# lazear/sage

Measured on NVIDIA H100. Metric: spectra/sec, higher is better.
Workload: dtype f32

## Files before the change

include/sage_b200.h:

```cpp
#ifndef SAGE_B200_H
#define SAGE_B200_H

#include <stddef.h>
#include <stdint.h>

#ifdef __cplusplus
extern "C" {
#endif

#define SAGE_B200_OK 0
#define SAGE_B200_EINVAL (-1)
#define SAGE_B200_ECUDA (-2)
#define SAGE_B200_ENOTMS2 (-3)
#define SAGE_B200_ENOPRECURSOR (-4)
#define SAGE_B200_ELIMIT (-5)

typedef struct sage_b200_db sage_b200_db;
typedef struct sage_b200_scorer sage_b200_scorer;

enum { SAGE_B200_TOL_PPM = 0, SAGE_B200_TOL_PCT = 1, SAGE_B200_TOL_DA = 2 };
typedef struct { int32_t kind; float lo, hi; } sage_b200_tolerance;

enum { SAGE_B200_KIND_A = 0, SAGE_B200_KIND_B = 1, SAGE_B200_KIND_C = 2, SAGE_B200_KIND_X = 3, SAGE_B200_KIND_Y = 4, SAGE_B200_KIND_Z = 5 };

// ... 101 lines not shown
int sage_b200_db_export_index(const sage_b200_db* db, uint32_t* fragment_peptide, float* fragment_mz, float* bucket_min);
void sage_b200_db_destroy(sage_b200_db* db);

int sage_b200_scorer_create(const sage_b200_db* db, const sage_b200_scorer_params* params, sage_b200_scorer** out);
void sage_b200_scorer_destroy(sage_b200_scorer* scorer);
int sage_b200_scorer_set_option(sage_b200_scorer* scorer, const char* name, int64_t value);

int sage_b200_score_batch(sage_b200_scorer* scorer, const sage_b200_spectra* spectra, sage_b200_feature* features, uint32_t* counts,
                          sage_b200_fragment* fragments, uint64_t fragment_capacity, uint64_t* fragments_used);

int sage_b200_score_batch_multi(sage_b200_scorer* const* scorers, int n_scorers, const sage_b200_spectra* spectra, sage_b200_feature* features,
                                uint32_t* counts);

int sage_b200_bind_thread_to_device(int device);

int sage_b200_quick_score(sage_b200_scorer* scorer, const sage_b200_spectra* spectra, int prefilter_low_memory, uint8_t* keep);

int sage_b200_batch_upload(sage_b200_scorer* scorer, const sage_b200_spectra* spectra);
int sage_b200_batch_run(sage_b200_scorer* scorer);
int sage_b200_batch_download(sage_b200_scorer* scorer, sage_b200_feature* features, uint32_t* counts);

int64_t sage_b200_initial_hits(sage_b200_scorer* scorer, const sage_b200_spectra* one_spectrum, uint16_t* matched, uint32_t* peptide,
                               uint8_t* charge, int8_t* isotope_error, uint64_t cap, uint64_t* matched_peaks, uint64_t* scored_candidates);

int sage_b200_counters_get(const sage_b200_scorer* scorer, sage_b200_counters* out);

typedef struct { uint64_t take_top_n; uint8_t deisotope; float min_deisotope_mz; } sage_b200_processor_params;
typedef struct {
    uint64_t n;
    const uint64_t* peak_offsets;
    const float* mz;
    const float* intensity;
    const uint8_t* precursor_charge;
    const uint8_t* level;
} sage_b200_raw_spectra;
int sage_b200_process_spectra(int device, const sage_b200_processor_params* processor, const sage_b200_raw_spectra* raw, uint64_t* out_peak_offsets,
                              float* out_masses, float* out_intensities, float* out_tic);

int sage_b200_find_reporter_ions(int device, uint64_t n, const uint64_t* peak_offsets, const float* masses, const float* intensities, const float* labels,
                                 uint64_t n_labels, sage_b200_tolerance label_tolerance, float* out);

int sage_b200_host_log_variant(void);
int sage_b200_host_log1pf_exact(void);
int sage_b200_device_log(int device, int variant, const double* x, uint64_t n, double* out);

typedef struct sage_b200_lfq sage_b200_lfq;
// ... 172 lines not shown
```

sage_b200/api.py:

```python
from __future__ import annotations

import ctypes as C
import os
from dataclasses import dataclass, field

import numpy as np

from .build import build_library, library_path

PPM, PCT, DA = 0, 1, 2
KIND = {"a": 0, "b": 1, "c": 2, "x": 3, "y": 4, "z": 5}


class SageB200Error(RuntimeError):
    def __init__(self, code: int, message: str):
        super().__init__(f"sage_b200 error {code}: {message}")
        self.code = code
        self.message = message


class CTol(C.Structure):
    _fields_ = [("kind", C.c_int32), ("lo", C.c_float), ("hi", C.c_float)]


# ... 28 lines not shown
COUNTER_U64 = ["spectra", "peaks", "queries", "tasks", "pages", "entries_scanned", "matched_fragments", "candidates_scored", "peptide_record_floats",
               "psms", "wide_queries", "pep_queries", "pep_fallbacks", "wide_overflows", "algorithmic_bytes", "prelim_bytes", "score_bytes", "h2d_bytes", "d2h_bytes", "kernel_launches", "chunk_retries"]
COUNTER_F32 = ["ms_total", "ms_h2d", "ms_setup", "ms_prelim", "ms_score", "ms_d2h", "ms_prelim_count", "ms_wall"]


class CCounters(C.Structure):
    _fields_ = [(n, C.c_uint64) for n in COUNTER_U64] + [(n, C.c_float) for n in COUNTER_F32]


FEATURE_DTYPE = np.dtype([
    ("spectrum", "<u4"), ("peptide_idx", "<u4"), ("peptide_len", "<u4"), ("rank", "<u4"), ("label", "<i4"), ("expmass", "<f4"), ("calcmass", "<f4"),
    ("charge", "<u4"), ("rt", "<f4"), ("ims", "<f4"), ("delta_mass", "<f4"), ("isotope_error", "<f4"), ("average_ppm", "<f4"), ("_pad0", "<u4"),
    ("hyperscore", "<f8"), ("delta_next", "<f8"), ("delta_best", "<f8"), ("matched_peaks", "<u4"), ("longest_b", "<u4"), ("longest_y", "<u4"),
    ("longest_y_pct", "<f4"), ("missed_cleavages", "<u4"), ("matched_intensity_pct", "<f4"), ("scored_candidates", "<u4"), ("ms2_intensity", "<f4"),
    ("poisson", "<f8"), ("fragment_offset", "<u4"), ("fragment_count", "<u4"),
])
assert FEATURE_DTYPE.itemsize == 128
FRAGMENT_DTYPE = np.dtype([("kind", "<i4"), ("charge", "<i4"), ("ordinal", "<i4"), ("intensity", "<f4"), ("mz_calculated", "<f4"),
                           ("mz_experimental", "<f4")])

EXPORTED_SYMBOLS = [
    "sage_b200_device_count", "sage_b200_db_create", "sage_b200_db_build", "sage_b200_db_get_info", "sage_b200_db_export_index", "sage_b200_db_destroy",
    "sage_b200_scorer_create", "sage_b200_scorer_destroy", "sage_b200_scorer_set_option", "sage_b200_score_batch", "sage_b200_batch_upload", "sage_b200_batch_run",
    "sage_b200_batch_download", "sage_b200_score_batch_multi", "sage_b200_quick_score", "sage_b200_initial_hits", "sage_b200_counters_get",
    "sage_b200_process_spectra", "sage_b200_find_reporter_ions", "sage_b200_host_alloc", "sage_b200_host_free", "sage_b200_last_error",
    "sage_b200_host_log_variant", "sage_b200_host_log1pf_exact", "sage_b200_device_log", "sage_b200_bind_thread_to_device", "sage_b200_host_alloc_blocks",
    "sage_b200_lfq_create", "sage_b200_lfq_add_ms1", "sage_b200_lfq_integrate", "sage_b200_lfq_get_info", "sage_b200_lfq_export", "sage_b200_lfq_destroy",
    "sage_b200_spectrum_fdr", "sage_b200_kde_build", "sage_b200_device_math", "sage_b200_predict_rt",
    "sage_b200_picked_fdr", "sage_b200_picked_precursor", "sage_b200_competition_keys", "sage_b200_protein_groups", "sage_b200_bipartite_cover",
]

_lib = None


def load_library(build: bool = True):
    global _lib
    if _lib is not None:
        return _lib
    path = library_path()
    if not os.path.exists(path):
        if not build:
            raise FileNotFoundError(f"{path} not built; run `python -m sage_b200.build`")
        build_library()
    lib = C.CDLL(path)
    for s in EXPORTED_SYMBOLS:
        getattr(lib, s)
    lib.sage_b200_host_alloc.restype = C.c_void_p
    lib.sage_b200_host_alloc.argtypes = [C.c_size_t]
    lib.sage_b200_host_free.argtypes = [C.c_void_p]
    lib.sage_b200_host_alloc_blocks.restype = C.c_void_p
    lib.sage_b200_host_alloc_blocks.argtypes = [C.c_size_t, C.c_void_p, C.c_int]
    lib.sage_b200_last_error.restype = C.c_size_t
    lib.sage_b200_initial_hits.restype = C.c_int64
    lib.sage_b200_db_destroy.argtypes = [C.c_void_p]
    lib.sage_b200_scorer_destroy.argtypes = [C.c_void_p]
    lib.sage_b200_lfq_destroy.argtypes = [C.c_void_p]
    _lib = lib
    return lib


def _last_error() -> str:
    buf = C.create_string_buffer(2048)
    load_library().sage_b200_last_error(buf, C.c_size_t(2048))
    return buf.value.decode(errors="replace")


def _check(rc: int):
    if rc != 0:
        raise SageB200Error(int(rc), _last_error())


def device_count() -> int:
    return int(load_library().sage_b200_device_count())


def bind_thread_to_device(device: int) -> int:
# ... 339 lines not shown
            keep = np.zeros(self.db.info["n_peptides"], np.uint8)
        keep_c = np.ascontiguousarray(keep, dtype=np.uint8)
        kl: list = []
        cs = batch._c(kl)
        _check(load_library().sage_b200_quick_score(self._h, C.byref(cs), C.c_int(int(prefilter_low_memory)), _ptr(keep_c)))
        return keep_c

    def score(self, spectrum: ProcessedSpectrum):
        out, counts = self.score_batch(SpectraBatch.from_spectra([spectrum]))
        return out[:counts[0]]

    def initial_hits(self, batch: SpectraBatch):
        assert len(batch) == 1
        cap = 256
        m, p = np.zeros(cap, np.uint16), np.zeros(cap, np.uint32)
        c, i = np.zeros(cap, np.uint8), np.zeros(cap, np.int8)
        mp, scd = C.c_uint64(0), C.c_uint64(0)
        keep: list = []
        cs = batch._c(keep)
        n = load_library().sage_b200_initial_hits(self._h, C.byref(cs), _ptr(m), _ptr(p), _ptr(c), _ptr(i), C.c_uint64(cap), C.byref(mp), C.byref(scd))
        if n < 0:
            raise SageB200Error(int(n), _last_error())
        return dict(matched=m[:n].copy(), peptide=p[:n].copy(), charge=c[:n].copy(), iso=i[:n].copy(), matched_peaks=mp.value, scored_candidates=scd.value)

    def counters(self) -> dict:
        cc = CCounters()
        _check(load_library().sage_b200_counters_get(self._h, C.byref(cc)))
        return {k: getattr(cc, k) for k, _ in CCounters._fields_}


def score_batch_multi(scorers, batch: SpectraBatch, out: np.ndarray | None = None, counts: np.ndarray | None = None):
    n, r = len(batch), scorers[0].report_psms
    if out is None:
        out = np.zeros(n * r, FEATURE_DTYPE)
    if counts is None:
        counts = np.zeros(n, np.uint32)
    keep: list = []
    cs = batch._c(keep)
    arr = (C.c_void_p * len(scorers))(*[s._h for s in scorers])
    _check(load_library().sage_b200_score_batch_multi(arr, C.c_int(len(scorers)), C.byref(cs), _ptr(out), _ptr(counts)))
    return out, counts


class CProcessorParams(C.Structure):
    _fields_ = [("take_top_n", C.c_uint64), ("deisotope", C.c_uint8), ("min_deisotope_mz", C.c_float)]

# ... 436 lines not shown
```

sage_b200/csrc/device_common.cuh:

```cuda
#pragma once
#include <cuda_runtime.h>
#include <stdint.h>

namespace sb {

constexpr int K_MAX = 128;
constexpr uint32_t NARROW_CAP = 8192;
constexpr int PRELIM_THREADS = 256;
constexpr int PRELIM_CTAS = 6;
constexpr int SCORE_THREADS = 128;
#ifndef SAGE_B200_SCORE_MIN_CTAS
#define SAGE_B200_SCORE_MIN_CTAS 10
#endif
constexpr int SCORE_MIN_CTAS = SAGE_B200_SCORE_MIN_CTAS;
#ifndef SAGE_B200_SCORE_TILE
#define SAGE_B200_SCORE_TILE 1024
#endif
#ifndef SAGE_B200_SCORE_UNROLL
#define SAGE_B200_SCORE_UNROLL 1
#endif
#ifndef SAGE_B200_SCORE_MIN_CTAS_SPLIT
#define SAGE_B200_SCORE_MIN_CTAS_SPLIT 11
#endif
constexpr int SCORE_MIN_CTAS_SPLIT = SAGE_B200_SCORE_MIN_CTAS_SPLIT;
// ... 49 lines not shown
    lo = left; hi = n;
    while (lo < hi) {
        uint32_t mid = lo + ((hi - lo) >> 1);
        if (le_hi(mid)) lo = mid + 1; else hi = mid;
    }
    right = lo;
}

__device__ __forceinline__ uint32_t max_fragment_charge(int opt, uint32_t precursor_charge) {
    uint32_t m = opt >= 0 ? (uint32_t)(opt + 1) : precursor_charge;
    m &= 0xFF;
    uint32_t r = precursor_charge < m ? precursor_charge : m;
    return r < 2 ? 2 : r;
}

__device__ __forceinline__ uint64_t prescore_key(uint32_t matched, uint32_t peptide, uint32_t charge, int iso) {
    return ((uint64_t)matched << 48) | ((uint64_t)peptide << 16) | ((uint64_t)(charge & 0xFF) << 8) | (uint64_t)((uint32_t)(iso + 128) & 0xFF);
}
constexpr uint64_t PRESCORE_DEFAULT = ((uint64_t)0xFFFFFFFFull << 16) | 128ull;
__device__ __forceinline__ uint32_t key_matched(uint64_t k) { return (uint32_t)(k >> 48); }
__device__ __forceinline__ uint32_t key_peptide(uint64_t k) { return (uint32_t)(k >> 16); }
__device__ __forceinline__ uint32_t key_charge(uint64_t k) { return (uint32_t)(k >> 8) & 0xFF; }
__device__ __forceinline__ int key_iso(uint64_t k) { return (int)(k & 0xFF) - 128; }

__device__ __forceinline__ void sift_down(uint64_t* s, uint32_t len, uint32_t index) {
    while (index * 2 + 1 < len) {
        uint32_t smallest = index, l = index * 2 + 1, r = index * 2 + 2;
        if (s[l] < s[smallest]) smallest = l;
        if (r < len && s[r] < s[smallest]) smallest = r;
        if (smallest != index) {
            uint64_t t = s[smallest]; s[smallest] = s[index]; s[index] = t;
            index = smallest;
        } else break;
    }
}
__device__ __forceinline__ void bounded_min_heapify_seq(uint64_t* s, uint32_t len, uint32_t k) {
    if (len <= k) return;
    for (uint32_t i = k / 2; i-- > 0;) sift_down(s, k, i);
    for (uint32_t i = k; i < len; i++) {
        if (s[i] > s[0]) {
            uint64_t t = s[i]; s[i] = s[0]; s[0] = t;
            sift_down(s, k, 0);
        }
    }
}

// ... 140 lines not shown
```

sage_b200/csrc/kernels.cuh:

```cuda
#pragma once
#include <type_traits>

#include "device_common.cuh"
#include "glibc_log.cuh"

#ifndef SAGE_B200_RARE_NOINLINE
#define SAGE_B200_RARE_NOINLINE 0
#endif
#if SAGE_B200_RARE_NOINLINE
#define SB_RARE __noinline__
#else
#define SB_RARE __forceinline__
#endif

namespace sb {

__device__ __forceinline__ uint32_t pep_partition(const DbView& db, float x, bool le) {
    uint32_t lo = 0, hi = db.n_pep;
    if (db.pep_lut != nullptr) {
        const float t = (x - db.plut_base) * db.plut_inv_w;
        if (t == t) {
            const int c = (int)fminf(fmaxf(floorf(t), -2.0f), (float)PEP_LUT_CELLS + 2.0f);
            lo = __ldg(db.pep_lut + min(max(c - 1, 0), (int)PEP_LUT_CELLS));
            hi = __ldg(db.pep_lut + min(max(c + 2, 0), (int)PEP_LUT_CELLS));
// ... 308 lines not shown
            const uint32_t e0 = __shfl_sync(0xffffffffu, e, src);
            const float lo_s = __shfl_sync(0xffffffffu, flo, src), hi_s = __shfl_sync(0xffffffffu, fhi, src);
            for (uint32_t pos = e0; pos < cnt; pos += 32) {
                const uint32_t i = pos + lane;
                bool stop = i >= cnt;
                if (!stop) {
                    const float fmz = __ldg(mz + i);
                    const uint32_t pid = pep0 + __ldg(off + i);
                    stop = fmz > hi_s;
                    if (!stop && fmz >= lo_s) {
                        if (pid >= q.eff_lo && pid <= q.eff_hi) {
                            const uint32_t idx = pid - q.pre_lo;
                            atomicAdd(&cnt32[idx >> 1], 1u << ((idx & 1) * 16));
                            matched++;
                        }
                    }
                }
                if (__any_sync(0xffffffffu, stop)) break;
            }
        }
    }
}

__device__ __forceinline__ void narrow_cta_query(const DbView& db, const ScorerView& sc, const BatchView& b, uint32_t pmax, uint64_t* nlist, uint32_t item,
                                                 float* bounds_smem, const NarrowIndexView& nv) {
    __shared__ uint32_t cnt32[NARROW_CAP / 2 + 1];
    __shared__ uint32_t s_warp[40];
    ReplaySlot* const nslots = b.nslots;
    const uint32_t s = item / sc.qmax;
    const QueryDesc q = b.queries[item];
    const uint32_t tid = threadIdx.x, lane = tid & 31, warp = tid >> 5, nwarps = PRELIM_THREADS / 32;
    const uint32_t p0 = b.peak_off[s], np = b.peak_off[s + 1] - p0;
    const uint32_t nwords = (q.potential + 1) >> 1;
    for (uint32_t i = tid; i < nwords; i += PRELIM_THREADS) cnt32[i] = 0;
    __shared__ unsigned long long s_loff;
    if (tid == 0 && q.potential > sc.kparam) s_loff = atomicAdd(b.counters + C_NLIST, (unsigned long long)q.potential);

    const uint32_t nfc = q.nfc;
    const uint32_t ntask = np * nfc;
    uint32_t my_matched = 0, my_pages = 0, my_entries = 0;
    __shared__ LutParams s_lp[8];
    bool pep_path = q.mode == 3 && np > 0 && np < 65536 && nfc <= 8;
    float* const bnd = bounds_smem;
    uint16_t* const luts = reinterpret_cast<uint16_t*>(bounds_smem + 2 * (size_t)nfc * pmax);
    if (pep_path) {
        for (uint32_t t = tid; t < ntask; t += PRELIM_THREADS) {
            const uint32_t c = t / np, p = t - c * np;
// ... 122 lines not shown
    uint32_t nzc = 0;
    if (n <= k) {
        uint64_t* keys = b.hit_keys + (size_t)item * sc.kparam;
        for (uint32_t i = tid; i < n; i += PRELIM_THREADS) {
            const uint32_t c = cnt(i);
            nzc += c != 0;
            keys[i] = c ? prescore_key(c, q.pre_lo + i, q.charge, q.iso) : PRESCORE_DEFAULT;
        }
        const uint32_t nzt = block_sum_u32(nzc, s_warp);
        if (tid == 0) {
            h->n = n; h->default_run = 0; h->matched_peaks = matched_total; h->scored_candidates = nzt;
            slot->off = 0; slot->item = item; slot->n_list = 0; slot->state = 1; slot->k = k;
        }
        return;
    }
    const unsigned long long loff = s_loff;
    if (loff + n > b.nlist_cap) {
        if (tid == 0) {
            h->n = 0; h->default_run = q.potential; h->matched_peaks = 0; h->scored_candidates = 0;
            slot->off = 0; slot->item = item; slot->n_list = 0; slot->state = 1; slot->k = 0;
        }
        return;
    }
    uint64_t* list = nlist + loff;
    for (uint32_t i = tid; i < k; i += PRELIM_THREADS) {
        const uint32_t c = cnt(i);
        nzc += c != 0;
        list[i] = c ? prescore_key(c, q.pre_lo + i, q.charge, q.iso) : PRESCORE_DEFAULT;
    }
    uint32_t wbase = k;
    for (uint32_t base = k; base < n; base += PRELIM_THREADS) {
        const uint32_t i = base + tid;
        const uint32_t c = i < n ? cnt(i) : 0;
        nzc += c != 0;
        const uint32_t ball = __ballot_sync(0xffffffffu, c != 0);
        if (lane == 0) s_warp[warp] = __popc(ball);
        __syncthreads();
        uint32_t off = 0, total = 0;
        for (uint32_t w = 0; w < nwarps; w++) {
            const uint32_t x = s_warp[w];
            if (w < warp) off += x;
            total += x;
        }
        if (c) list[wbase + off + __popc(ball & ((1u << lane) - 1))] = prescore_key(c, q.pre_lo + i, q.charge, q.iso);
        wbase += total;
        __syncthreads();
    }
    const uint32_t nzt = block_sum_u32(nzc, s_warp);
    if (tid == 0) {
        h->n = k; h->default_run = 0; h->matched_peaks = matched_total; h->scored_candidates = nzt;
        slot->off = loff; slot->item = item; slot->n_list = wbase; slot->state = 0; slot->k = k;
    }
}

__global__ void __launch_bounds__(PRELIM_THREADS, PRELIM_CTAS) k_prelim_narrow(DbView db, ScorerView sc, BatchView b, uint32_t pmax, uint64_t* nlist, NarrowIndexView nv) {
    extern __shared__ float bounds_smem[];
    const uint32_t total = (uint32_t)min(b.counters[C_NCTA], (unsigned long long)b.n * sc.qmax);
    for (uint32_t i = blockIdx.x; i < total; i += gridDim.x) {
        narrow_cta_query(db, sc, b, pmax, nlist, b.cta_items[i], bounds_smem, nv);
        __syncthreads();
    }
}

template <bool BLK>
__global__ void __launch_bounds__(WARPQ_WARPS * 32, WARPQ_MIN_CTAS) k_prelim_narrow_warp(DbView db, ScorerView sc, BatchView b, uint64_t* nlist, uint32_t s_lo,
                                                                                                uint32_t s_hi, NarrowIndexView nv) {
    __shared__ uint32_t cnt_all[WARPQ_WARPS][WARPQ_CAP / 2];
    if (b.counters[C_COUNT + blockIdx.y] == 0ull) return;
    const uint32_t lane = threadIdx.x & 31, warp = threadIdx.x >> 5;
    const uint32_t pos = blockIdx.x * WARPQ_WARPS + warp;
    if (pos >= b.n) return;
    const uint32_t s = b.order ? b.order[pos] : pos;
    if (s < s_lo || s >= s_hi) return;
    const uint32_t item = s * sc.qmax + blockIdx.y;
    const QueryDesc q = b.queries[item];
    if (q.mode != 4) return;
    uint32_t* const cnt32 = cnt_all[warp];
    const uint32_t n = q.potential, k = min(n, sc.kparam);
    for (uint32_t i = lane; i < (n + 1) >> 1; i += 32) cnt32[i] = 0;
    unsigned long long loff = 0;
    if (n > k) {
        if (lane == 0) loff = atomicAdd(b.counters + C_NLIST, (unsigned long long)n);
        loff = __shfl_sync(0xffffffffu, loff, 0);
    }
    __syncwarp();
    const uint32_t p0 = b.peak_off[s], np = b.peak_off[s + 1] - p0;
    const uint32_t nfc = q.nfc, ntask = np * nfc;
    uint32_t matched = 0, pages = 0, entries = 0;
// ... 9 lines not shown
        }
        if (BLK) block_probe_warp(nv, q, blk0, blk1, act, flo, fhi, cnt32, matched);
        else if (act) index_probe(db, q, flo, fhi, cnt32, matched, pages, entries);
    }
    for (int o = 16; o > 0; o >>= 1) {
        matched += __shfl_xor_sync(0xffffffffu, matched, o);
        pages += __shfl_xor_sync(0xffffffffu, pages, o);
        entries += __shfl_xor_sync(0xffffffffu, entries, o);
    }
    __syncwarp();
    if (lane == 0) {
        atomicAdd(b.counters + C_TASKS, (unsigned long long)ntask);
        if (pages) atomicAdd(b.counters + C_PAGES, (unsigned long long)pages);
        if (entries) atomicAdd(b.counters + C_ENTRIES, (unsigned long long)entries);
        if (matched) atomicAdd(b.counters + C_MATCHED, (unsigned long long)matched);
    }
    QueryHits* h = b.hits + item;
    ReplaySlot* slot = b.nslots + item;
    if (matched == 0 || (n > k && loff + n > b.nlist_cap)) {
        if (lane == 0) { h->n = 0; h->default_run = n; h->matched_peaks = 0; h->scored_candidates = 0; }
        return;
    }
    auto cnt = [&](uint32_t i) -> uint32_t { return (cnt32[i >> 1] >> ((i & 1) * 16)) & 0xFFFFu; };
    uint32_t nzc = 0;
    uint64_t* dst = n <= k ? b.hit_keys + (size_t)item * sc.kparam : nlist + loff;
    for (uint32_t i = lane; i < k; i += 32) {
        const uint32_t c = cnt(i);
        nzc += c != 0;
        dst[i] = c ? prescore_key(c, q.pre_lo + i, q.charge, q.iso) : PRESCORE_DEFAULT;
    }
    uint32_t wbase = k;
    for (uint32_t base = k; base < n; base += 32) {
        const uint32_t i = base + lane;
        const uint32_t c = i < n ? cnt(i) : 0;
        nzc += c != 0;
        const uint32_t ball = __ballot_sync(0xffffffffu, c != 0);
        if (c) dst[wbase + __popc(ball & ((1u << lane) - 1))] = prescore_key(c, q.pre_lo + i, q.charge, q.iso);
        wbase += __popc(ball);
    }
    for (int o = 16; o > 0; o >>= 1) nzc += __shfl_xor_sync(0xffffffffu, nzc, o);
    if (lane == 0) {
        h->n = k; h->default_run = 0; h->matched_peaks = matched; h->scored_candidates = nzc;
        if (n > k) { slot->off = loff; slot->n_list = wbase; slot->state = 0; slot->k = k; }
    }
}

#ifndef SAGE_B200_WIDE_THREADS
#define SAGE_B200_WIDE_THREADS 512
#endif
#ifndef SAGE_B200_WIDE_TILE
#define SAGE_B200_WIDE_TILE (32 * 1024)
#endif
#ifndef SAGE_B200_WIDE_CTAS
#define SAGE_B200_WIDE_CTAS 2
#endif
constexpr int WIDE_THREADS = SAGE_B200_WIDE_THREADS;
constexpr int WIDE_CTAS = SAGE_B200_WIDE_CTAS;
constexpr bool WIDE_SMALL = WIDE_CTAS > 1;
constexpr uint32_t WIDE_TILE = SAGE_B200_WIDE_TILE;
constexpr uint32_t WIDE_VMAX = WIDE_SMALL ? 1024 : 2048;
constexpr uint32_t WIDE_TCACHE = WIDE_SMALL ? 1024 : 2048;
// ... 586 lines not shown
        tol_bounds(sc.fragment_tol, mass, flo, fhi);
        uint32_t bl, br;
        bucket_range(db, flo, fhi, bl, br);
        for (uint32_t page = bl; page < br; page++) {
            const uint64_t pbase = (uint64_t)page * db.bucket_size;
            const uint32_t pn = (uint32_t)(min(pbase + db.bucket_size, db.n_frag) - pbase);
            const uint32_t st = page_lower_bound_dir(db, page, db.frag + pbase, pn, q.pre_lo);
            const uint32_t en = page_lower_bound_dir(db, page, db.frag + pbase, pn, q.pre_hi + 1);
            entries += en - (st == 0 ? 0 : st - 1);
            pages++;
        }
    }
    for (int o = 16; o > 0; o >>= 1) {
        pages += __shfl_down_sync(0xffffffffu, pages, o);
        entries += __shfl_down_sync(0xffffffffu, entries, o);
    }
    if (lane == 0) {
        if (pages) atomicAdd(b.counters + C_PAGES, pages);
        if (entries) atomicAdd(b.counters + C_ENTRIES, entries);
    }
}

constexpr int REPLAY_THREADS = 128;
template <bool COMPACT>
__global__ void __launch_bounds__(REPLAY_THREADS) k_replay(ScorerView sc, BatchView b, const uint64_t* lists, const ReplaySlot* slots, uint32_t n_slots,
                                                           const unsigned long long* n_slots_dev, uint32_t n_spectra) {
    typedef typename std::conditional<COMPACT, uint32_t, uint64_t>::type key_t;
    extern __shared__ __align__(8) unsigned char rheap_raw[];
    key_t* const rheap = reinterpret_cast<key_t*>(rheap_raw);
    uint32_t slot = blockIdx.x * REPLAY_THREADS + threadIdx.x;
    if (n_slots_dev != nullptr) n_slots = (uint32_t)min((unsigned long long)n_slots, *n_slots_dev);
    if (slot >= n_slots) return;
    if (n_spectra) { const uint32_t pos = slot % n_spectra; slot = (b.order ? b.order[pos] : pos) * sc.qmax + slot / n_spectra; }
    const ReplaySlot ws = slots[slot];
    if (ws.state != 0) return;
    const uint64_t* list = lists + ws.off;
    const uint32_t k = ws.k, tid = threadIdx.x;
    uint32_t pre_lo = 0, q_charge = 0;
    int q_iso = 0;
    if (COMPACT) { const QueryDesc q = b.queries[ws.item]; pre_lo = q.pre_lo; q_charge = q.charge; q_iso = q.iso; }
    auto pack = [&](uint64_t k64) -> key_t {
        if (!COMPACT) return (key_t)k64;
        return (key_t)(key_peptide(k64) == 0xFFFFFFFFu ? 0x0000FFFFu : ((key_matched(k64) << 16) | (key_peptide(k64) - pre_lo)));
    };
    auto unpack = [&](key_t kk) -> uint64_t {
        if (!COMPACT) return (uint64_t)kk;
        const uint32_t v = (uint32_t)kk;
        return v == 0x0000FFFFu ? PRESCORE_DEFAULT : prescore_key(v >> 16, pre_lo + (v & 0xFFFFu), q_charge, q_iso);
    };
    auto H = [&](uint32_t i) -> key_t& { return rheap[i * REPLAY_THREADS + tid]; };
    auto sift = [&](uint32_t index, key_t val) {
        for (;;) {
            const uint32_t l = index * 2 + 1;
            if (l >= k) break;
            uint32_t c = l;
            key_t cv = H(l);
            if (l + 1 < k) { const key_t cr = H(l + 1); if (cr < cv) { cv = cr; c = l + 1; } }
            if (!(cv < val)) break;
            H(index) = cv;
            index = c;
        }
        H(index) = val;
    };
    for (uint32_t i = 0; i < k; i++) H(i) = pack(__ldg(list + i));
    for (uint32_t i = k / 2; i-- > 0;) sift(i, H(i));
    key_t root = H(0);
    uint64_t nxt = k < ws.n_list ? __ldg(list + k) : 0;
    for (uint32_t j = k; j < ws.n_list; j++) {
        const key_t kq = pack(nxt);
        if (j + 1 < ws.n_list) nxt = __ldg(list + j + 1);
        if (kq > root) { sift(0, kq); root = H(0); }
    }
    uint64_t* keys = b.hit_keys + (size_t)ws.item * sc.kparam;
    for (uint32_t i = 0; i < k; i++) keys[i] = unpack(H(i));
}

struct ScoreRec {
    double hyperscore;
    uint32_t peptide;
    uint32_t matched_b, matched_y;
    float summed_b, summed_y;
    uint32_t longest_b, longest_y;
    float ppm_difference;
    uint32_t charge;
    int iso;
    uint32_t valid;
    uint32_t plen;
};

__device__ SB_RARE int select_most_intense_peak(const float* masses, const float* intens, uint32_t n, float center, const Tol& tol) {
    float lo, hi;
    tol_bounds(tol, center, lo, hi);
    lo = __fadd_rn(lo, 0.0f);
    hi = __fadd_rn(hi, 0.0f);
    const int klo = f32_key(lo), khi = f32_key(hi);
    uint32_t i, j;
    binary_search_slice(n, [&](uint32_t k) { return f32_key(masses[k]) < klo; }, [&](uint32_t k) { return f32_key(masses[k]) <= khi; }, i, j);
// ... 1365 lines not shown
```

sage_b200/csrc/sage_b200.cu:

```cuda
#include <cub/device/device_radix_sort.cuh>
#include <cub/device/device_scan.cuh>
#include <cub/device/device_select.cuh>
#include <cub/device/device_reduce.cuh>
#include <cub/device/device_merge_sort.cuh>
#include <cub/device/device_run_length_encode.cuh>
#include <cub/device/device_segmented_sort.cuh>
#include <cuda_runtime.h>
#include <thrust/iterator/counting_iterator.h>

#include <pthread.h>
#include <sched.h>

#include <algorithm>
#include <atomic>
#include <cctype>
#include <cmath>
#include <cstdarg>
#include <cstdio>
#include <cstdlib>
#include <cstring>
#include <limits>
#include <chrono>
#include <condition_variable>
#include <memory>
// ... 1200 lines not shown
        CUDA_TRY(cudaMemcpyAsync(L.d_counters.as<unsigned long long>() + C_FRAGS, hbase, 8, cudaMemcpyHostToDevice, st));
    }
    ScorerView svq = sv;
    uint32_t mfc = sv.max_fragment_charge_opt >= 0 ? std::min<uint32_t>(C.zmax, (uint32_t)(sv.max_fragment_charge_opt + 1) & 0xFF) : C.zmax;
    if (mfc < 2) mfc = 2;
    size_t pep_smem = (size_t)(mfc - 1) * (2 * (size_t)C.pmax * sizeof(float) + 2 * LUT_CELLS * sizeof(uint16_t));
    if (mfc - 1 > 8) pep_smem = 200 * 1024;
    if (pep_smem > 96 * 1024) { svq.pep_cap = 0; pep_smem = 0; }
    if (svq.pep_cap == 0) pep_smem = 0;
    uint32_t *sk_in = nullptr, *sk_out = nullptr, *sv_in = nullptr, *sv_out = nullptr;
    int sort_bits = 1;
    while (sort_bits < 32 && (db->v.n_pep >> sort_bits)) sort_bits++;
    const int sort_lo = std::max(0, sort_bits - 16);
    size_t sort_tmp = 0;
    if (S->sort_spectra && n > 1) {
        if ((rc = L.d_sort.reserve(16 * (size_t)n))) return rc;
        sk_in = L.d_sort.as<uint32_t>(); sk_out = sk_in + n; sv_in = sk_out + n; sv_out = sv_in + n;
        CUDA_TRY(cub::DeviceRadixSort::SortPairs(nullptr, sort_tmp, sk_in, sk_out, sv_in, sv_out, (int)n, sort_lo, sort_bits, st));
        if ((rc = L.d_sorttmp.reserve(sort_tmp + 16))) return rc;
    }
    C.nlist_cap = std::max<uint64_t>(C.force_nlist, (uint64_t)std::ceil(S->nlist_per_spectrum * (double)n) + 4096);
    C.wide_cap = (uint32_t)std::min<uint64_t>(C.nitems, std::max<uint64_t>(C.force_wide, S->wide_per_spectrum > 0.0
                                                                               ? (uint64_t)std::ceil(S->wide_per_spectrum * 1.1 * (double)n) + 64 : 0));
    if ((rc = L.d_nlist.reserve(8 * (C.nlist_cap + 16)))) return rc;
    if ((rc = L.d_nslots.reserve(C.nitems * sizeof(ReplaySlot)))) return rc;
    if (C.wide_cap) {
        if ((rc = L.d_witems.reserve(4 * (size_t)C.wide_cap))) return rc;
        if ((rc = L.d_wlist.reserve((size_t)C.wide_cap * WIDE_LMAX * 8))) return rc;
        if ((rc = L.d_wslots.reserve((size_t)C.wide_cap * sizeof(WideSlot)))) return rc;
    }
    if ((rc = L.d_citems.reserve(4 * C.nitems))) return rc;
    bv.cta_items = L.d_citems.as<uint32_t>();
    bv.nslots = L.d_nslots.as<ReplaySlot>();
    bv.wide_items = L.d_witems.as<uint32_t>();
    bv.wide_cap = C.wide_cap;
    bv.nlist_cap = C.nlist_cap;
    k_setup_queries<<<(n + 127) / 128, 128, 0, st>>>(db->v, svq, bv, sk_in, sv_in);
    CUDA_TRY(cudaGetLastError());
    if (sk_in) {
        CUDA_TRY(cub::DeviceRadixSort::SortPairs(L.d_sorttmp.p, sort_tmp, sk_in, sk_out, sv_in, sv_out, (int)n, sort_lo, sort_bits, st));
        bv.order = sv_out;
    }
    CUDA_TRY(cudaEventRecord(L.ev_setup_end, st));
    if (C.nparts <= 1) CUDA_TRY(cudaStreamWaitEvent(st, L.ev_masses, 0));
    uint64_t launches = 1;

    const size_t rsm = (size_t)sv.kparam * REPLAY_THREADS * 8;
    const float ptol_span = std::max(std::fabs(sv.precursor_tol.lo), std::fabs(sv.precursor_tol.hi));
    const bool narrow_tol = ptol_span <= (sv.precursor_tol.kind == 0 ? 2000.0f : sv.precursor_tol.kind == 1 ? 0.2f : 5.0f);
    NarrowIndexView nv{};
    if (S->narrow_index && !sv.wide_window && narrow_tol) {
        if (S->narrow_block == 0 && (rc = narrow_block_for(S))) return rc;
        nv = db_narrow_index(db, S->narrow_block ? S->narrow_block : S->narrow_block_auto, S->narrow_block != 0);
    }
    for (uint32_t q = 0; q < C.nparts; q++) {
        if (C.nparts > 1) CUDA_TRY(cudaStreamWaitEvent(st, L.ev_part[q], 0));
        const dim3 wgrid((n + WARPQ_WARPS - 1) / WARPQ_WARPS, sv.qmax);
        if (nv.mz != nullptr) k_prelim_narrow_warp<true><<<wgrid, WARPQ_WARPS * 32, 0, st>>>(db->v, svq, bv, L.d_nlist.as<uint64_t>(), C.part_lo[q], C.part_lo[q + 1], nv);
        else k_prelim_narrow_warp<false><<<wgrid, WARPQ_WARPS * 32, 0, st>>>(db->v, svq, bv, L.d_nlist.as<uint64_t>(), C.part_lo[q], C.part_lo[q + 1], nv);
        CUDA_TRY(cudaGetLastError());
        launches += q > 0;
    }
    if (C.nparts > 1) CUDA_TRY(cudaStreamWaitEvent(st, L.ev_masses, 0));
    k_prelim_narrow<<<(unsigned)std::min<uint64_t>(C.nitems, (uint64_t)db->sm_count * PRELIM_CTAS), PRELIM_THREADS, pep_smem, st>>>(db->v, svq, bv, C.pmax, L.d_nlist.as<uint64_t>(),
                                                                                                                         S->narrow_cta ? nv : NarrowIndexView{});
    CUDA_TRY(cudaGetLastError());
    CUDA_TRY(cudaEventRecord(L.ev_count_end, st));
    k_replay<true><<<(unsigned)((C.nitems + REPLAY_THREADS - 1) / REPLAY_THREADS), REPLAY_THREADS, rsm / 2, st>>>(sv, bv, L.d_nlist.as<uint64_t>(), L.d_nslots.as<ReplaySlot>(),
                                                                                                                 (uint32_t)C.nitems, nullptr, n);
    CUDA_TRY(cudaGetLastError());
    launches += 3;
    if (C.wide_cap) {
        const int ctas = (int)std::min<uint64_t>((uint64_t)db->sm_count * WIDE_CTAS, C.wide_cap);
        const WideIndexView wv = db_wide_index(db, sv.wide_tile);
        k_prelim_wide<<<ctas, WIDE_THREADS, sizeof(WideSmem), st>>>(db->v, sv, bv, (uint32_t)C.nitems, L.d_wlist.as<uint64_t>(), L.d_wslots.as<WideSlot>(), wv);
        CUDA_TRY(cudaGetLastError());
        if (wv.frag != nullptr) {
            k_wide_account<<<(C.wide_cap + 7) / 8, 256, 0, st>>>(db->v, sv, bv);
            CUDA_TRY(cudaGetLastError());
            launches++;
        }
        k_replay<false><<<(unsigned)((C.wide_cap + REPLAY_THREADS - 1) / REPLAY_THREADS), REPLAY_THREADS, rsm, st>>>(
            sv, bv, L.d_wlist.as<uint64_t>(), L.d_wslots.as<WideSlot>(), C.wide_cap, L.d_counters.as<unsigned long long>() + C_WIDE, 0u);
        CUDA_TRY(cudaGetLastError());
        launches += 2;
    }
    CUDA_TRY(cudaEventRecord(L.ev_replay_end, st));

    if ((rc = lane_join_stager(L))) return rc;
    CUDA_TRY(cudaStreamWaitEvent(st, L.ev_intens, 0));
    const bool split = S->score_split && !sv.chimera && !annotate && !dbg && S->quick_mode == 0;
    if (split) {
// ... 465 lines not shown
    std::vector<sage_b200_feature> f(S->sv.report_psms);
    uint32_t cnt = 0;
    Lane& L = S->lanes[0];
    if ((rc = chunk_upload(S, L, sp, 0, 1))) return rc;
    if ((rc = chunk_run(S, L, true))) return rc;
    if ((rc = chunk_download(S, L, f.data(), &cnt))) return rc;
    if ((rc = lane_finish(S, L))) return rc;
    L.chunk.loaded = false;
    std::vector<uint64_t> keys(S->sv.kparam);
    uint32_t meta[4] = {0, 0, 0, 0};
    CUDA_TRY(cudaMemcpy(keys.data(), L.d_dbgk.p, 8 * (size_t)S->sv.kparam, cudaMemcpyDeviceToHost));
    CUDA_TRY(cudaMemcpy(meta, L.d_dbgm.p, 16, cudaMemcpyDeviceToHost));
    const uint32_t nk = meta[0];
    for (uint32_t i = 0; i < nk && i < cap; i++) {
        const uint64_t k = keys[i];
        if (matched) matched[i] = (uint16_t)(k >> 48);
        if (peptide) peptide[i] = (uint32_t)(k >> 16);
        if (charge) charge[i] = (uint8_t)(k >> 8);
        if (isotope_error) isotope_error[i] = (int8_t)((int)(k & 0xFF) - 128);
    }
    if (matched_peaks) *matched_peaks = meta[1];
    if (scored_candidates) *scored_candidates = meta[2];
    return (int64_t)nk;
}

extern "C" int sage_b200_process_spectra(int device, const sage_b200_processor_params* pr, const sage_b200_raw_spectra* raw, uint64_t* out_peak_offsets,
                                         float* out_masses, float* out_intensities, float* out_tic) {
    if (!pr || !raw || !out_peak_offsets || !out_tic) return fail(SAGE_B200_EINVAL, "process_spectra: null argument");
    if (int rc = select_device(device)) return rc;
    cudaGetLastError();
    const uint64_t n = raw->n;
    out_peak_offsets[0] = 0;
    if (n == 0) return 0;
    if (!raw->peak_offsets || !raw->precursor_charge) return fail(SAGE_B200_EINVAL, "process_spectra: null array");
    const uint64_t pk0 = raw->peak_offsets[0], npk = raw->peak_offsets[n] - pk0;
    if (npk && (!raw->mz || !raw->intensity || !out_masses || !out_intensities)) return fail(SAGE_B200_EINVAL, "process_spectra: null peak arrays");
    if (n > 0x7FFFFFFFull || npk > 0xFFFFFFF0ull) return fail(SAGE_B200_ELIMIT, "process_spectra: batch too large");
    std::vector<uint32_t> off(n + 1);
    uint32_t pmax = 1;
    for (uint64_t i = 0; i <= n; i++) off[i] = (uint32_t)(raw->peak_offsets[i] - pk0);
    for (uint64_t i = 0; i < n; i++) {
        if (raw->level && raw->level[i] != 2) return fail(SAGE_B200_ENOTMS2, "process_spectra handles MS2 spectra only (spectrum %llu has level %u)", (unsigned long long)i, raw->level[i]);
        pmax = std::max(pmax, off[i + 1] - off[i]);
    }
    uint32_t p2 = 1;
    while (p2 < pmax) p2 <<= 1;
// ... 2018 lines not shown
```

Measured before the change: 26.09 million.

## Store narrow candidate lists as 32-bit compact keys and warp-stage replay loads

The narrow prelim kernels now write 32-bit compact keys (matched count and peptide offset) into the candidate list instead of full 64-bit prescore keys, which halves list memory traffic and allocation. The compact replay kernel is restructured so each warp cooperatively loads rounds of its lanes' lists with coalesced loads into padded shared memory, and each thread then runs its heap selection from shared memory using vector reads. Block size and round are exposed as compile-time knobs. A debug API is also added that exports per-slot list lengths. The trade-offs are extra shared memory and warp-level divergence, since every lane iterates up to the longest list in its warp.

```diff
diff --git a/include/sage_b200.h b/include/sage_b200.h
--- a/include/sage_b200.h
+++ b/include/sage_b200.h
@@ -147,6 +147,8 @@
 
 int64_t sage_b200_initial_hits(sage_b200_scorer* scorer, const sage_b200_spectra* one_spectrum, uint16_t* matched, uint32_t* peptide,
                                uint8_t* charge, int8_t* isotope_error, uint64_t cap, uint64_t* matched_peaks, uint64_t* scored_candidates);
+
+int64_t sage_b200_replay_lists(sage_b200_scorer* scorer, uint32_t* n_list, uint64_t cap);
 
 int sage_b200_counters_get(const sage_b200_scorer* scorer, sage_b200_counters* out);
 
diff --git a/sage_b200/api.py b/sage_b200/api.py
--- a/sage_b200/api.py
+++ b/sage_b200/api.py
@@ -74,7 +74,7 @@
 EXPORTED_SYMBOLS = [
     "sage_b200_device_count", "sage_b200_db_create", "sage_b200_db_build", "sage_b200_db_get_info", "sage_b200_db_export_index", "sage_b200_db_destroy",
     "sage_b200_scorer_create", "sage_b200_scorer_destroy", "sage_b200_scorer_set_option", "sage_b200_score_batch", "sage_b200_batch_upload", "sage_b200_batch_run",
-    "sage_b200_batch_download", "sage_b200_score_batch_multi", "sage_b200_quick_score", "sage_b200_initial_hits", "sage_b200_counters_get",
+    "sage_b200_batch_download", "sage_b200_score_batch_multi", "sage_b200_quick_score", "sage_b200_initial_hits", "sage_b200_replay_lists", "sage_b200_counters_get",
     "sage_b200_process_spectra", "sage_b200_find_reporter_ions", "sage_b200_host_alloc", "sage_b200_host_free", "sage_b200_last_error",
     "sage_b200_host_log_variant", "sage_b200_host_log1pf_exact", "sage_b200_device_log", "sage_b200_bind_thread_to_device", "sage_b200_host_alloc_blocks",
     "sage_b200_lfq_create", "sage_b200_lfq_add_ms1", "sage_b200_lfq_integrate", "sage_b200_lfq_get_info", "sage_b200_lfq_export", "sage_b200_lfq_destroy",
@@ -104,6 +104,7 @@
     lib.sage_b200_host_alloc_blocks.argtypes = [C.c_size_t, C.c_void_p, C.c_int]
     lib.sage_b200_last_error.restype = C.c_size_t
     lib.sage_b200_initial_hits.restype = C.c_int64
+    lib.sage_b200_replay_lists.restype = C.c_int64
     lib.sage_b200_db_destroy.argtypes = [C.c_void_p]
     lib.sage_b200_scorer_destroy.argtypes = [C.c_void_p]
     lib.sage_b200_lfq_destroy.argtypes = [C.c_void_p]
@@ -489,6 +490,16 @@
         if n < 0:
             raise SageB200Error(int(n), _last_error())
         return dict(matched=m[:n].copy(), peptide=p[:n].copy(), charge=c[:n].copy(), iso=i[:n].copy(), matched_peaks=mp.value, scored_candidates=scd.value)
+
+    def replay_lists(self) -> np.ndarray:
+        n = load_library().sage_b200_replay_lists(self._h, None, C.c_uint64(0))
+        if n < 0:
+            raise SageB200Error(int(n), _last_error())
+        out = np.zeros(n, np.uint32)
+        n = load_library().sage_b200_replay_lists(self._h, _ptr(out), C.c_uint64(len(out)))
+        if n < 0:
+            raise SageB200Error(int(n), _last_error())
+        return out
 
     def counters(self) -> dict:
         cc = CCounters()
diff --git a/sage_b200/csrc/device_common.cuh b/sage_b200/csrc/device_common.cuh
--- a/sage_b200/csrc/device_common.cuh
+++ b/sage_b200/csrc/device_common.cuh
@@ -95,6 +95,10 @@
 __device__ __forceinline__ uint32_t key_peptide(uint64_t k) { return (uint32_t)(k >> 16); }
 __device__ __forceinline__ uint32_t key_charge(uint64_t k) { return (uint32_t)(k >> 8) & 0xFF; }
 __device__ __forceinline__ int key_iso(uint64_t k) { return (int)(k & 0xFF) - 128; }
+__device__ __forceinline__ uint32_t compact_key(uint32_t matched, uint32_t offset) { return matched ? (matched << 16) | offset : 0x0000FFFFu; }
+__device__ __forceinline__ uint64_t expand_compact_key(uint32_t v, uint32_t pre_lo, uint32_t charge, int iso) {
+    return v == 0x0000FFFFu ? PRESCORE_DEFAULT : prescore_key(v >> 16, pre_lo + (v & 0xFFFFu), charge, iso);
+}
 
 __device__ __forceinline__ void sift_down(uint64_t* s, uint32_t len, uint32_t index) {
     while (index * 2 + 1 < len) {
diff --git a/sage_b200/csrc/kernels.cuh b/sage_b200/csrc/kernels.cuh
--- a/sage_b200/csrc/kernels.cuh
+++ b/sage_b200/csrc/kernels.cuh
@@ -354,7 +354,7 @@
     }
 }
 
-__device__ __forceinline__ void narrow_cta_query(const DbView& db, const ScorerView& sc, const BatchView& b, uint32_t pmax, uint64_t* nlist, uint32_t item,
+__device__ __forceinline__ void narrow_cta_query(const DbView& db, const ScorerView& sc, const BatchView& b, uint32_t pmax, uint32_t* nlist, uint32_t item,
                                                  float* bounds_smem, const NarrowIndexView& nv) {
     __shared__ uint32_t cnt32[NARROW_CAP / 2 + 1];
     __shared__ uint32_t s_warp[40];
@@ -523,11 +523,11 @@
         }
         return;
     }
-    uint64_t* list = nlist + loff;
+    uint32_t* list = nlist + loff;
     for (uint32_t i = tid; i < k; i += PRELIM_THREADS) {
         const uint32_t c = cnt(i);
         nzc += c != 0;
-        list[i] = c ? prescore_key(c, q.pre_lo + i, q.charge, q.iso) : PRESCORE_DEFAULT;
+        list[i] = compact_key(c, i);
     }
     uint32_t wbase = k;
     for (uint32_t base = k; base < n; base += PRELIM_THREADS) {
@@ -543,7 +543,7 @@
             if (w < warp) off += x;
             total += x;
         }
-        if (c) list[wbase + off + __popc(ball & ((1u << lane) - 1))] = prescore_key(c, q.pre_lo + i, q.charge, q.iso);
+        if (c) list[wbase + off + __popc(ball & ((1u << lane) - 1))] = compact_key(c, i);
         wbase += total;
         __syncthreads();
     }
@@ -554,7 +554,7 @@
     }
 }
 
-__global__ void __launch_bounds__(PRELIM_THREADS, PRELIM_CTAS) k_prelim_narrow(DbView db, ScorerView sc, BatchView b, uint32_t pmax, uint64_t* nlist, NarrowIndexView nv) {
+__global__ void __launch_bounds__(PRELIM_THREADS, PRELIM_CTAS) k_prelim_narrow(DbView db, ScorerView sc, BatchView b, uint32_t pmax, uint32_t* nlist, NarrowIndexView nv) {
     extern __shared__ float bounds_smem[];
     const uint32_t total = (uint32_t)min(b.counters[C_NCTA], (unsigned long long)b.n * sc.qmax);
     for (uint32_t i = blockIdx.x; i < total; i += gridDim.x) {
@@ -564,7 +564,7 @@
 }
 
 template <bool BLK>
-__global__ void __launch_bounds__(WARPQ_WARPS * 32, WARPQ_MIN_CTAS) k_prelim_narrow_warp(DbView db, ScorerView sc, BatchView b, uint64_t* nlist, uint32_t s_lo,
+__global__ void __launch_bounds__(WARPQ_WARPS * 32, WARPQ_MIN_CTAS) k_prelim_narrow_warp(DbView db, ScorerView sc, BatchView b, uint32_t* nlist, uint32_t s_lo,
                                                                                                 uint32_t s_hi, NarrowIndexView nv) {
     __shared__ uint32_t cnt_all[WARPQ_WARPS][WARPQ_CAP / 2];
     if (b.counters[C_COUNT + blockIdx.y] == 0ull) return;
@@ -620,21 +620,29 @@
         return;
     }
     auto cnt = [&](uint32_t i) -> uint32_t { return (cnt32[i >> 1] >> ((i & 1) * 16)) & 0xFFFFu; };
-    uint32_t nzc = 0;
-    uint64_t* dst = n <= k ? b.hit_keys + (size_t)item * sc.kparam : nlist + loff;
-    for (uint32_t i = lane; i < k; i += 32) {
-        const uint32_t c = cnt(i);
-        nzc += c != 0;
-        dst[i] = c ? prescore_key(c, q.pre_lo + i, q.charge, q.iso) : PRESCORE_DEFAULT;
-    }
-    uint32_t wbase = k;
-    for (uint32_t base = k; base < n; base += 32) {
-        const uint32_t i = base + lane;
-        const uint32_t c = i < n ? cnt(i) : 0;
-        nzc += c != 0;
-        const uint32_t ball = __ballot_sync(0xffffffffu, c != 0);
-        if (c) dst[wbase + __popc(ball & ((1u << lane) - 1))] = prescore_key(c, q.pre_lo + i, q.charge, q.iso);
-        wbase += __popc(ball);
+    uint32_t nzc = 0, wbase = k;
+    if (n <= k) {
+        uint64_t* keys = b.hit_keys + (size_t)item * sc.kparam;
+        for (uint32_t i = lane; i < n; i += 32) {
+            const uint32_t c = cnt(i);
+            nzc += c != 0;
+            keys[i] = c ? prescore_key(c, q.pre_lo + i, q.charge, q.iso) : PRESCORE_DEFAULT;
+        }
+    } else {
+        uint32_t* list = nlist + loff;
+        for (uint32_t i = lane; i < k; i += 32) {
+            const uint32_t c = cnt(i);
+            nzc += c != 0;
+            list[i] = compact_key(c, i);
+        }
+        for (uint32_t base = k; base < n; base += 32) {
+            const uint32_t i = base + lane;
+            const uint32_t c = i < n ? cnt(i) : 0;
+            nzc += c != 0;
+            const uint32_t ball = __ballot_sync(0xffffffffu, c != 0);
+            if (c) list[wbase + __popc(ball & ((1u << lane) - 1))] = compact_key(c, i);
+            wbase += __popc(ball);
+        }
     }
     for (int o = 16; o > 0; o >>= 1) nzc += __shfl_xor_sync(0xffffffffu, nzc, o);
     if (lane == 0) {
@@ -1267,33 +1275,32 @@
 }
 
 constexpr int REPLAY_THREADS = 128;
+#ifndef SAGE_B200_REPLAY_THREADS
+#define SAGE_B200_REPLAY_THREADS 64
+#endif
+#ifndef SAGE_B200_REPLAY_ROUND
+#define SAGE_B200_REPLAY_ROUND 64
+#endif
+constexpr int NREPLAY_THREADS = SAGE_B200_REPLAY_THREADS;
+constexpr int NREPLAY_ROUND = SAGE_B200_REPLAY_ROUND;
+constexpr int NREPLAY_PITCH = NREPLAY_ROUND + 4;
+constexpr uint32_t NREPLAY_BATCH = 16;
+static_assert(NREPLAY_THREADS % 32 == 0 && NREPLAY_ROUND % 32 == 0, "the staging loads cover a round in whole warps");
+__host__ __device__ constexpr size_t replay_narrow_smem(uint32_t kparam) {
+    return (size_t)NREPLAY_THREADS * NREPLAY_PITCH * 4 + (size_t)kparam * NREPLAY_THREADS * 4;
+}
 template <bool COMPACT>
-__global__ void __launch_bounds__(REPLAY_THREADS) k_replay(ScorerView sc, BatchView b, const uint64_t* lists, const ReplaySlot* slots, uint32_t n_slots,
-                                                           const unsigned long long* n_slots_dev, uint32_t n_spectra) {
+__global__ void __launch_bounds__(COMPACT ? NREPLAY_THREADS : REPLAY_THREADS)
+k_replay(ScorerView sc, BatchView b, const typename std::conditional<COMPACT, uint32_t, uint64_t>::type* lists, const ReplaySlot* slots,
+         uint32_t n_slots, const unsigned long long* n_slots_dev, uint32_t n_spectra) {
     typedef typename std::conditional<COMPACT, uint32_t, uint64_t>::type key_t;
-    extern __shared__ __align__(8) unsigned char rheap_raw[];
-    key_t* const rheap = reinterpret_cast<key_t*>(rheap_raw);
-    uint32_t slot = blockIdx.x * REPLAY_THREADS + threadIdx.x;
-    if (n_slots_dev != nullptr) n_slots = (uint32_t)min((unsigned long long)n_slots, *n_slots_dev);
-    if (slot >= n_slots) return;
-    if (n_spectra) { const uint32_t pos = slot % n_spectra; slot = (b.order ? b.order[pos] : pos) * sc.qmax + slot / n_spectra; }
-    const ReplaySlot ws = slots[slot];
-    if (ws.state != 0) return;
-    const uint64_t* list = lists + ws.off;
-    const uint32_t k = ws.k, tid = threadIdx.x;
-    uint32_t pre_lo = 0, q_charge = 0;
-    int q_iso = 0;
-    if (COMPACT) { const QueryDesc q = b.queries[ws.item]; pre_lo = q.pre_lo; q_charge = q.charge; q_iso = q.iso; }
-    auto pack = [&](uint64_t k64) -> key_t {
-        if (!COMPACT) return (key_t)k64;
-        return (key_t)(key_peptide(k64) == 0xFFFFFFFFu ? 0x0000FFFFu : ((key_matched(k64) << 16) | (key_peptide(k64) - pre_lo)));
-    };
-    auto unpack = [&](key_t kk) -> uint64_t {
-        if (!COMPACT) return (uint64_t)kk;
-        const uint32_t v = (uint32_t)kk;
-        return v == 0x0000FFFFu ? PRESCORE_DEFAULT : prescore_key(v >> 16, pre_lo + (v & 0xFFFFu), q_charge, q_iso);
-    };
-    auto H = [&](uint32_t i) -> key_t& { return rheap[i * REPLAY_THREADS + tid]; };
+    constexpr uint32_t T = COMPACT ? NREPLAY_THREADS : REPLAY_THREADS;
+    extern __shared__ __align__(16) unsigned char rheap_raw[];
+    key_t* const rheap = reinterpret_cast<key_t*>(rheap_raw + (COMPACT ? (size_t)NREPLAY_THREADS * NREPLAY_PITCH * 4 : 0));
+    uint32_t slot = blockIdx.x * T + threadIdx.x;
+    const uint32_t tid = threadIdx.x;
+    auto H = [&](uint32_t i) -> key_t& { return rheap[i * T + tid]; };
+    uint32_t k = 0;
     auto sift = [&](uint32_t index, key_t val) {
         for (;;) {
             const uint32_t l = index * 2 + 1;
@@ -1307,17 +1314,84 @@
         }
         H(index) = val;
     };
-    for (uint32_t i = 0; i < k; i++) H(i) = pack(__ldg(list + i));
-    for (uint32_t i = k / 2; i-- > 0;) sift(i, H(i));
-    key_t root = H(0);
-    uint64_t nxt = k < ws.n_list ? __ldg(list + k) : 0;
-    for (uint32_t j = k; j < ws.n_list; j++) {
-        const key_t kq = pack(nxt);
-        if (j + 1 < ws.n_list) nxt = __ldg(list + j + 1);
-        if (kq > root) { sift(0, kq); root = H(0); }
-    }
-    uint64_t* keys = b.hit_keys + (size_t)ws.item * sc.kparam;
-    for (uint32_t i = 0; i < k; i++) keys[i] = unpack(H(i));
+    if constexpr (COMPACT) {
+        const uint32_t lane = tid & 31;
+        uint32_t n = 0, item = 0;
+        unsigned long long off = 0;
+        if (slot < n_slots) {
+            const uint32_t pos = slot % n_spectra;
+            slot = (b.order ? b.order[pos] : pos) * sc.qmax + slot / n_spectra;
+            const ReplaySlot ws = slots[slot];
+            if (ws.state == 0) { n = ws.n_list; k = ws.k; item = ws.item; off = ws.off; }
+        }
+        const uint32_t nmax = __reduce_max_sync(0xffffffffu, n);
+        if (nmax == 0) return;
+        uint32_t* const stage = reinterpret_cast<uint32_t*>(rheap_raw) + (tid & ~31u) * NREPLAY_PITCH;
+        const uint32_t* const mine = stage + lane * NREPLAY_PITCH;
+        key_t root = 0;
+        for (uint32_t p0 = 0; p0 < nmax; p0 += NREPLAY_ROUND) {
+            for (uint32_t L0 = 0; L0 < 32; L0 += NREPLAY_BATCH) {
+                uint32_t v[NREPLAY_BATCH][NREPLAY_ROUND / 32];
+#pragma unroll
+                for (uint32_t u = 0; u < NREPLAY_BATCH; u++) {
+                    const uint32_t nL = __shfl_sync(0xffffffffu, n, L0 + u);
+                    const unsigned long long oL = __shfl_sync(0xffffffffu, off, L0 + u);
+#pragma unroll
+                    for (uint32_t c = 0; c < NREPLAY_ROUND / 32; c++)
+                        v[u][c] = p0 + c * 32 + lane < nL ? __ldg(lists + oL + p0 + c * 32 + lane) : 0u;
+                }
+#pragma unroll
+                for (uint32_t u = 0; u < NREPLAY_BATCH; u++)
+#pragma unroll
+                    for (uint32_t c = 0; c < NREPLAY_ROUND / 32; c++) stage[(L0 + u) * NREPLAY_PITCH + c * 32 + lane] = v[u][c];
+            }
+            __syncwarp();
+            const uint32_t m = p0 < n ? min((uint32_t)NREPLAY_ROUND, n - p0) : 0;
+            for (uint32_t r = 0; r < m; r += 4) {
+                const uint4 v4 = *reinterpret_cast<const uint4*>(mine + r);
+                const uint32_t kv[4] = {v4.x, v4.y, v4.z, v4.w};
+#pragma unroll
+                for (uint32_t u = 0; u < 4; u++) {
+                    const uint32_t j = p0 + r + u;
+                    if (r + u >= m) break;
+                    const key_t kq = kv[u];
+                    if (j < k) {
+                        H(j) = kq;
+                        if (j + 1 == k) {
+                            for (uint32_t i = k / 2; i-- > 0;) sift(i, H(i));
+                            root = H(0);
+                        }
+                    } else if (kq > root) {
+                        sift(0, kq);
+                        root = H(0);
+                    }
+                }
+            }
+            __syncwarp();
+        }
+        if (n == 0) return;
+        const QueryDesc q = b.queries[item];
+        uint64_t* keys = b.hit_keys + (size_t)item * sc.kparam;
+        for (uint32_t i = 0; i < k; i++) keys[i] = expand_compact_key(H(i), q.pre_lo, q.charge, q.iso);
+    } else {
+        if (n_slots_dev != nullptr) n_slots = (uint32_t)min((unsigned long long)n_slots, *n_slots_dev);
+        if (slot >= n_slots) return;
+        const ReplaySlot ws = slots[slot];
+        if (ws.state != 0) return;
+        const uint64_t* list = lists + ws.off;
+        k = ws.k;
+        for (uint32_t i = 0; i < k; i++) H(i) = __ldg(list + i);
+        for (uint32_t i = k / 2; i-- > 0;) sift(i, H(i));
+        key_t root = H(0);
+        uint64_t nxt = k < ws.n_list ? __ldg(list + k) : 0;
+        for (uint32_t j = k; j < ws.n_list; j++) {
+            const key_t kq = nxt;
+            if (j + 1 < ws.n_list) nxt = __ldg(list + j + 1);
+            if (kq > root) { sift(0, kq); root = H(0); }
+        }
+        uint64_t* keys = b.hit_keys + (size_t)ws.item * sc.kparam;
+        for (uint32_t i = 0; i < k; i++) keys[i] = H(i);
+    }
 }
 
 struct ScoreRec {
diff --git a/sage_b200/csrc/sage_b200.cu b/sage_b200/csrc/sage_b200.cu
--- a/sage_b200/csrc/sage_b200.cu
+++ b/sage_b200/csrc/sage_b200.cu
@@ -1246,7 +1246,7 @@
     C.nlist_cap = std::max<uint64_t>(C.force_nlist, (uint64_t)std::ceil(S->nlist_per_spectrum * (double)n) + 4096);
     C.wide_cap = (uint32_t)std::min<uint64_t>(C.nitems, std::max<uint64_t>(C.force_wide, S->wide_per_spectrum > 0.0
                                                                                ? (uint64_t)std::ceil(S->wide_per_spectrum * 1.1 * (double)n) + 64 : 0));
-    if ((rc = L.d_nlist.reserve(8 * (C.nlist_cap + 16)))) return rc;
+    if ((rc = L.d_nlist.reserve(4 * (C.nlist_cap + 16)))) return rc;
     if ((rc = L.d_nslots.reserve(C.nitems * sizeof(ReplaySlot)))) return rc;
     if (C.wide_cap) {
         if ((rc = L.d_witems.reserve(4 * (size_t)C.wide_cap))) return rc;
@@ -1280,18 +1280,18 @@
     for (uint32_t q = 0; q < C.nparts; q++) {
         if (C.nparts > 1) CUDA_TRY(cudaStreamWaitEvent(st, L.ev_part[q], 0));
         const dim3 wgrid((n + WARPQ_WARPS - 1) / WARPQ_WARPS, sv.qmax);
-        if (nv.mz != nullptr) k_prelim_narrow_warp<true><<<wgrid, WARPQ_WARPS * 32, 0, st>>>(db->v, svq, bv, L.d_nlist.as<uint64_t>(), C.part_lo[q], C.part_lo[q + 1], nv);
-        else k_prelim_narrow_warp<false><<<wgrid, WARPQ_WARPS * 32, 0, st>>>(db->v, svq, bv, L.d_nlist.as<uint64_t>(), C.part_lo[q], C.part_lo[q + 1], nv);
+        if (nv.mz != nullptr) k_prelim_narrow_warp<true><<<wgrid, WARPQ_WARPS * 32, 0, st>>>(db->v, svq, bv, L.d_nlist.as<uint32_t>(), C.part_lo[q], C.part_lo[q + 1], nv);
+        else k_prelim_narrow_warp<false><<<wgrid, WARPQ_WARPS * 32, 0, st>>>(db->v, svq, bv, L.d_nlist.as<uint32_t>(), C.part_lo[q], C.part_lo[q + 1], nv);
         CUDA_TRY(cudaGetLastError());
         launches += q > 0;
     }
     if (C.nparts > 1) CUDA_TRY(cudaStreamWaitEvent(st, L.ev_masses, 0));
-    k_prelim_narrow<<<(unsigned)std::min<uint64_t>(C.nitems, (uint64_t)db->sm_count * PRELIM_CTAS), PRELIM_THREADS, pep_smem, st>>>(db->v, svq, bv, C.pmax, L.d_nlist.as<uint64_t>(),
+    k_prelim_narrow<<<(unsigned)std::min<uint64_t>(C.nitems, (uint64_t)db->sm_count * PRELIM_CTAS), PRELIM_THREADS, pep_smem, st>>>(db->v, svq, bv, C.pmax, L.d_nlist.as<uint32_t>(),
                                                                                                                          S->narrow_cta ? nv : NarrowIndexView{});
     CUDA_TRY(cudaGetLastError());
     CUDA_TRY(cudaEventRecord(L.ev_count_end, st));
-    k_replay<true><<<(unsigned)((C.nitems + REPLAY_THREADS - 1) / REPLAY_THREADS), REPLAY_THREADS, rsm / 2, st>>>(sv, bv, L.d_nlist.as<uint64_t>(), L.d_nslots.as<ReplaySlot>(),
-                                                                                                                 (uint32_t)C.nitems, nullptr, n);
+    k_replay<true><<<(unsigned)((C.nitems + NREPLAY_THREADS - 1) / NREPLAY_THREADS), NREPLAY_THREADS, replay_narrow_smem(sv.kparam), st>>>(
+        sv, bv, L.d_nlist.as<uint32_t>(), L.d_nslots.as<ReplaySlot>(), (uint32_t)C.nitems, nullptr, n);
     CUDA_TRY(cudaGetLastError());
     launches += 3;
     if (C.wide_cap) {
@@ -1803,6 +1803,28 @@
     if (matched_peaks) *matched_peaks = meta[1];
     if (scored_candidates) *scored_candidates = meta[2];
     return (int64_t)nk;
+}
+
+extern "C" int64_t sage_b200_replay_lists(sage_b200_scorer* S, uint32_t* n_list, uint64_t cap) {
+    if (!S || (!n_list && cap)) return fail(SAGE_B200_EINVAL, "replay_lists: null argument");
+    std::lock_guard<std::mutex> lock(S->mu);
+    CUDA_TRY(cudaSetDevice(S->db->device));
+    Lane& L = S->lanes[0];
+    const ChunkState& C = L.chunk;
+    if (!C.loaded || C.nitems == 0 || L.d_nslots.cap < C.nitems * sizeof(ReplaySlot))
+        return fail(SAGE_B200_EINVAL, "replay_lists: no resident batch has run (call batch_upload and batch_run first)");
+    CUDA_TRY(cudaStreamSynchronize(L.stream));
+    std::vector<ReplaySlot> slots(C.nitems);
+    CUDA_TRY(cudaMemcpy(slots.data(), L.d_nslots.p, C.nitems * sizeof(ReplaySlot), cudaMemcpyDeviceToHost));
+    std::vector<uint32_t> order(C.n);
+    for (uint32_t i = 0; i < C.n; i++) order[i] = i;
+    if (S->sort_spectra && C.n > 1)
+        CUDA_TRY(cudaMemcpy(order.data(), L.d_sort.as<uint32_t>() + 3 * (size_t)C.n, 4 * (size_t)C.n, cudaMemcpyDeviceToHost));
+    for (uint64_t t = 0; t < C.nitems && t < cap; t++) {
+        const ReplaySlot& r = slots[(size_t)order[t % C.n] * S->sv.qmax + t / C.n];
+        n_list[t] = r.state == 0 ? r.n_list : 0;
+    }
+    return (int64_t)C.nitems;
 }
 
 extern "C" int sage_b200_process_spectra(int device, const sage_b200_processor_params* pr, const sage_b200_raw_spectra* raw, uint64_t* out_peak_offsets,
```

New measurement: 26.56 million (median of 6 runs). 1.8% higher.
